# Image-Processing-Systems-Laboratory/DeepInPainting

Measured on AMD Instinct MI355X. Metric: train images/sec at 256x256, batch 8/GPU, 1/2/4/8 MI355X; IPSR layer ms, higher is better.
Workload: dtype f32; 1 GPU; BASELINE config 2: 256x256 synthetic images, 128x128 centre mask (M=256 of N=1024 feature positions), batch 8/GPU, fp32, full IPSR training step; global_batch=8, parallelism=dp1, dropout=True, conv_math=fp32, vgg16=seeded random init (no pretrained weights offline)

## Files before the change

deepinpainting_amd/csrc/winograd.hip:

```cpp
#include <type_traits>

#include "ipsr_common.h"

namespace ipsr {

typedef float f32x16 __attribute__((ext_vector_type(16)));
typedef const __attribute__((address_space(1))) void* gptr_t;
typedef __attribute__((address_space(3))) void* lptr_t;

constexpr int WG_BM = 128, WG_BN = 128, WG_BK = 16, WG_NBUF = 4, WG_THREADS = 256;

struct WinoSplit {
    int nsplit, sps, xi_split, nsplit_t, sps_t;
    int nxi = 36;
    __host__ __device__ int slabs() const { return xi_split >= nxi ? nsplit : (xi_split <= 0 ? nsplit_t : (nsplit > nsplit_t ? nsplit : nsplit_t)); }
    __host__ __device__ int of(int xi) const { return xi < xi_split ? nsplit : nsplit_t; }
    __host__ __device__ int head_xi() const { return xi_split < nxi ? xi_split : nxi; }
    __host__ int workgroups(int tiles_per_xi) const { return tiles_per_xi * (head_xi() * nsplit + (nxi - head_xi()) * nsplit_t); }
};

__device__ __forceinline__ void wino_load_sum(const float* __restrict__ M, const WinoSplit sp, size_t plane, size_t off, float m[6][6])
{
#pragma unroll
    for (int i = 0; i < 6; ++i)
// ... 1104 lines not shown
        for (int j = 0; j < 3; ++j) {
            const int yy = 3 * ty + i, xx = 3 * tx + j;
            e[i][j] = (live && yy < Ho && xx < Wo) ? ld1(dp, (size_t)yy * Wo + xx) : 0.0f;
        }
    float w[6][3], v[6][6];
#pragma unroll
    for (int j = 0; j < 3; ++j) {
        const float col[3] = {e[0][j], e[1][j], e[2][j]};
        float o[6];
        wino_g(col, o);
#pragma unroll
        for (int i = 0; i < 6; ++i) w[i][j] = o[i];
    }
#pragma unroll
    for (int i = 0; i < 6; ++i) wino_g(w[i], v[i]);
    op_emit<true, MODE>(smem, v, ix, Et, Kp, Tp);
    }
};

__global__ void __launch_bounds__(256) wino_wrw_output4_kernel(const float* __restrict__ Mw, WinoSplit split, int K, int C, int Kp, int Cp,
                                                               float* __restrict__ dW)
{
    const int c = blockIdx.x * 256 + threadIdx.x, k = blockIdx.y;
    if (c >= C) return;
    float m[6][6];
    const size_t plane = (size_t)Kp * Cp;
    wino_load_sum(Mw, split, plane, (size_t)k * Cp + c, m);
    float w[4][6], o[4][4];
#pragma unroll
    for (int j = 0; j < 6; ++j) {
        const float col[6] = {m[0][j], m[1][j], m[2][j], m[3][j], m[4][j], m[5][j]};
        float r4[4];
        wino_at(col, r4);
#pragma unroll
        for (int i = 0; i < 4; ++i) w[i][j] = r4[i];
    }
#pragma unroll
    for (int i = 0; i < 4; ++i) wino_at(w[i], o[i]);
    float4* dst = reinterpret_cast<float4*>(dW + ((size_t)k * C + c) * 16);
#pragma unroll
    for (int i = 0; i < 4; ++i) dst[i] = make_float4(o[i][0], o[i][1], o[i][2], o[i][3]);
}

struct DilGrid { int Ho, Wo, Gy, Gx; };
static DilGrid dil_grid(int geom, int mode, int H, int W)
{
    const int Ho = geom == 0 ? H / 2 : H - 1, Wo = geom == 0 ? W / 2 : W - 1;
    return DilGrid{Ho, Wo, (geom == 1 && mode == 1) ? H : Ho, (geom == 1 && mode == 1) ? W : Wo};
}

static int dil_plan(int geom, int mode, int B, int Cin, int H, int W, int Cout, WinoGemmPlan* p, int math)
{
    if (geom != 0 && geom != 1) return fail(IPSR_ERR_INVALID, "4x4 winograd: geometry %d", geom);
    if (geom == 0 && ((H | W) & 1)) return fail(IPSR_ERR_UNSUPPORTED, "dilated winograd: odd extent %dx%d", H, W);
    if (geom == 1 && (H < 4 || W < 4)) return fail(IPSR_ERR_UNSUPPORTED, "4x4 winograd: extent %dx%d below the kernel", H, W);
    const DilGrid g = dil_grid(geom, mode, H, W);
    wino_plan_tiles(p, B, (g.Gy + 2) / 3, (g.Gx + 2) / 3);
    const int red = mode == 0 ? Cin : Cout;
    if (mode != 2 && red % WG_BK != 0)
        return fail(IPSR_ERR_UNSUPPORTED, "4x4 winograd: %d reduction channels are not a multiple of %d", red, WG_BK);
    if (mode == 2) wino_plan_gemm(p, Cout, round_up_bn(Cin), p->Tp, math);
    else wino_plan_gemm(p, mode == 0 ? Cout : Cin, p->Tp, red, math);
    return IPSR_OK;
}

size_t winograd_dil_ws_bytes(int geom, int mode, int B, int Cin, int H, int W, int Cout)
{
    return wino_ws_bytes([&](WinoGemmPlan* p, int math) { return dil_plan(geom, mode, B, Cin, H, W, Cout, p, math); });
}

template <bool TMAJOR, int MODE, typename T, typename F>
static void with_window3(int is, const T* x, int B, int C, int H, int W, int off, const WinoGemmPlan& p, int Cp, void* V, F&& f)
{
    const dim3 grid = op_grid(TMAJOR, MODE, p.Tp, TMAJOR ? Cp : C);
    if (is == 2) f(WinoWindow<3, 2, TMAJOR, MODE, T>{x, B, C, H, W, off, p.TY, p.TX, p.Tp, Cp, V}, grid);
    else f(WinoWindow<3, 1, TMAJOR, MODE, T>{x, B, C, H, W, off, p.TY, p.TX, p.Tp, Cp, V}, grid);
}

int launch_winograd_dil(int geom, int mode, const void* a, const void* b2, void* out, int B, int Cin, int H, int W, int Cout,
                        void* ws, size_t ws_bytes, hipStream_t st, ConvArith ar = ConvArith{0, false, false})
{
    WinoGemmPlan p;
    WinoBufs m;
    if (int rc = dil_plan(geom, mode, B, Cin, H, W, Cout, &p, ar.math)) return rc;
    if (int rc = wino_launch_head("4x4 winograd", "", p, ar, ws, ws_bytes, &m)) return rc;
    const DilGrid g = dil_grid(geom, mode, H, W);
    const int Ho = g.Ho, Wo = g.Wo;
    const int xis = geom == 0 ? 2 : 1, xoff = geom == 0 ? -3 : -1;
    if (mode == 0 || mode == 1) {
        const int red = mode == 0 ? Cin : Cout, prod = mode == 0 ? Cout : Cin;
        if (mode == 1 && geom == 0 && hipMemsetAsync(out, 0, (size_t)B * Cin * H * W * (ar.out_bf16 ? 2 : 4), st) != hipSuccess)
            return fail(IPSR_ERR_LAUNCH, "dilated winograd: hipMemsetAsync failed");
        const float* w = static_cast<const float*>(b2);
        with_mode(ar.math, [&](auto M) {
            constexpr int MODE = decltype(M)::value;
            const Wino4Filter<MODE> filt = mode == 0 ? Wino4Filter<MODE>{w, Cin, Cout, p.rows, 16, (long)Cin * 16, 0, m.A}
                                                     : Wino4Filter<MODE>{w, Cout, Cin, p.rows, (long)Cin * 16, 16, 1, m.A};
            const dim3 fgrid = op_grid(false, MODE, p.rows, red);
            with_type(ar.in_bf16, [&](auto* tag) {
                using T = ELEM_T(tag);
                auto go = [&](const auto& win, dim3 grid) { launch_pair(st, win, grid, wino_remap(), filt, fgrid); };
                if (mode == 0) with_window3<false, MODE, T>(xis, static_cast<const T*>(a), B, Cin, H, W, xoff, p, 0, m.B, go);
                else with_window3<false, MODE, T>(1, static_cast<const T*>(a), B, Cout, Ho, Wo, geom == 0 ? -1 : -2, p, 0, m.B, go);
            });
        });
        if (int rc = check_launch("wino_pair_kernel<WinoWindow, Wino4Filter>")) return rc;
        if (int rc = launch_wino_gemm(ar.math, p, m, st, 72.0 * red * prod * p.T)) return rc;
        with_type(ar.out_bf16, [&](auto* tag) {
            using T = ELEM_T(tag);
            if (mode == 0) wino3_output_kernel<T><<<dim3(cdiv(p.T, 256), prod), 256, 0, st>>>(m.M, p.sp, B, Cout, p.rows, Ho, Wo, p.TY, p.TX, p.Tp, Ho, Wo, 1, 0, static_cast<T*>(out));
            else wino3_output_kernel<T><<<dim3(cdiv(p.T, 256), prod), 256, 0, st>>>(m.M, p.sp, B, Cin, p.rows, g.Gy, g.Gx, p.TY, p.TX, p.Tp, H, W,
                                                                                    geom == 0 ? 2 : 1, geom == 0 ? 1 : 0, static_cast<T*>(out));
        });
        return check_launch("wino3_output_kernel");
    }
    with_mode(ar.math, [&](auto M) {
        constexpr int MODE = decltype(M)::value;
        with_type(ar.in_bf16, [&](auto* tag) {
            using T = ELEM_T(tag);
            const WinoWrwTile3<MODE, T> tile{static_cast<const T*>(b2), B, Cout, Ho, Wo, p.TY, p.TX, p.Tp, p.rows, m.A};
            with_window3<true, MODE, T>(xis, static_cast<const T*>(a), B, Cin, H, W, xoff, p, p.cols, m.B, [&](const auto& win, dim3 grid) {
                launch_pair_wrw(st, tile, op_grid(true, MODE, p.Tp, p.rows), win, grid, MODE != 3);
            });
        });
    });
    if (int rc = check_launch("wino_pair_kernel<WinoWrwTile3, WinoWindow>")) return rc;
    if (int rc = launch_wino_gemm(ar.math, p, m, st, 72.0 * p.T * Cout * Cin)) return rc;
    wino_wrw_output4_kernel<<<dim3(cdiv(Cin, 256), Cout), 256, 0, st>>>(m.M, p.sp, Cout, Cin, p.rows, p.cols, static_cast<float*>(out));
    return check_launch("wino_wrw_output4_kernel");
}

__device__ __forceinline__ void wino_g2(const float g[2], float u[6])
{
    u[0] = 0.25f * g[0];
    u[1] = (-1.0f / 6.0f) * (g[0] + g[1]);
    u[2] = (-1.0f / 6.0f) * (g[0] - g[1]);
    u[3] = (1.0f / 24.0f) * g[0] + (1.0f / 12.0f) * g[1];
    u[4] = (1.0f / 24.0f) * g[0] - (1.0f / 12.0f) * g[1];
    u[5] = g[1];
}
__device__ __forceinline__ void wino_at5(const float m[6], float y[5])
{
    y[0] = m[0] + m[1] + m[2] + m[3] + m[4];
    y[1] = m[1] - m[2] + 2.0f * m[3] - 2.0f * m[4];
    y[2] = m[1] + m[2] + 4.0f * m[3] + 4.0f * m[4];
    y[3] = m[1] - m[2] + 8.0f * m[3] - 8.0f * m[4];
    y[4] = m[1] + m[2] + 16.0f * m[3] + 16.0f * m[4] + m[5];
}
__device__ __forceinline__ void wino_g5(const float e[5], float u[6])
{
    u[0] = 0.25f * e[0];
    u[1] = (-1.0f / 6.0f) * (e[0] + e[1] + e[2] + e[3] + e[4]);
    u[2] = (-1.0f / 6.0f) * (e[0] - e[1] + e[2] - e[3] + e[4]);
    u[3] = (1.0f / 24.0f) * e[0] + (1.0f / 12.0f) * e[1] + (1.0f / 6.0f) * e[2] + (1.0f / 3.0f) * e[3] + (2.0f / 3.0f) * e[4];
    u[4] = (1.0f / 24.0f) * e[0] - (1.0f / 12.0f) * e[1] + (1.0f / 6.0f) * e[2] - (1.0f / 3.0f) * e[3] + (2.0f / 3.0f) * e[4];
    u[5] = e[4];
}
__device__ __forceinline__ void wino_at2(const float m[6], float y[2])
{
    y[0] = m[0] + m[1] + m[2] + m[3] + m[4];
    y[1] = m[1] - m[2] + 2.0f * m[3] - 2.0f * m[4] + m[5];
}

struct Wino52Filter {
    const float* W; int Kc, Cf, Qp, form; float* Uout;
    static constexpr int SMEM = 16;
    __device__ __forceinline__ void operator()(unsigned char*, unsigned bx, unsigned by) const
    {
    float* __restrict__ U = Uout;
    const int fast = bx * 256 + threadIdx.x, slow = by;
    const int nfast = form == 0 ? Kc : Cf;
    const int R = form == 0 ? 4 * Cf : Kc, Q = form == 0 ? Kc : 4 * Cf;
    const size_t plane = (size_t)R * Qp;
    if (fast >= nfast) {
        if (form == 0) {
            if (fast < Qp)
                for (int ph = 0; ph < 4; ++ph)
                    for (int xi = 0; xi < 36; ++xi) U[(size_t)xi * plane + (size_t)(ph * Cf + slow) * Qp + fast] = 0.0f;
        } else {
            const int q = Q + (fast - nfast);
            if (q < Qp)
                for (int xi = 0; xi < 36; ++xi) U[(size_t)xi * plane + (size_t)slow * Qp + q] = 0.0f;
        }
        return;
    }
    const int kc = form == 0 ? fast : slow, cf = form == 0 ? slow : fast;
    float w[4][4];
    const float4* wp = reinterpret_cast<const float4*>(W + ((size_t)kc * Cf + cf) * 16);
#pragma unroll
    for (int i = 0; i < 4; ++i) { const float4 v = wp[i]; w[i][0] = v.x; w[i][1] = v.y; w[i][2] = v.z; w[i][3] = v.w; }
#pragma unroll
    for (int ph = 0; ph < 4; ++ph) {
        const int ey = ph >> 1, ex = ph & 1;
        float g[2][2];
#pragma unroll
        for (int a = 0; a < 2; ++a)
#pragma unroll
            for (int b = 0; b < 2; ++b) g[a][b] = form == 0 ? w[2 * a + ey][2 * b + ex] : w[3 - ey - 2 * a][3 - ex - 2 * b];
        float t[6][2], u[6][6];
#pragma unroll
        for (int b = 0; b < 2; ++b) {
            const float col[2] = {g[0][b], g[1][b]};
            float o[6];
            wino_g2(col, o);
#pragma unroll
            for (int i = 0; i < 6; ++i) t[i][b] = o[i];
        }
#pragma unroll
        for (int i = 0; i < 6; ++i) wino_g2(t[i], u[i]);
        const size_t r = form == 0 ? (size_t)ph * Cf + cf : kc, q = form == 0 ? kc : (size_t)ph * Cf + cf;
#pragma unroll
        for (int i = 0; i < 6; ++i)
#pragma unroll
            for (int j = 0; j < 6; ++j) U[(size_t)(i * 6 + j) * plane + r * Qp + q] = u[i][j];
    }
    }
};

template <int NPL>
struct Wino52FilterSplit {
    const float* W; int Kc, Cf, Qp, form; unsigned short* U;
    static constexpr int SMEM = split_stage_elems<NPL>() * 2;
    __device__ __forceinline__ void operator()(unsigned char* smem, unsigned bx, unsigned by) const
    {
    unsigned short* stage = reinterpret_cast<unsigned short*>(smem);
    const int pk = threadIdx.x >> 5, rl = threadIdx.x & 31;
    const int kc = form == 0 ? bx * SPLIT_ROWS + rl : by * 8 + pk;
    const int cf = form == 0 ? by * 8 + pk : bx * SPLIT_ROWS + rl;
    const bool live = kc < Kc && cf < Cf;
    float w[4][4];
    const float4* wp = reinterpret_cast<const float4*>(W + ((size_t)(live ? kc : 0) * Cf + (live ? cf : 0)) * 16);
#pragma unroll
    for (int i = 0; i < 4; ++i) {
        const float4 v = live ? wp[i] : make_float4(0.f, 0.f, 0.f, 0.f);
        w[i][0] = v.x; w[i][1] = v.y; w[i][2] = v.z; w[i][3] = v.w;
    }
#pragma unroll
    for (int ph = 0; ph < 4; ++ph) {
        const int ey = ph >> 1, ex = ph & 1;
        float g[2][2];
#pragma unroll
        for (int a = 0; a < 2; ++a)
#pragma unroll
            for (int b = 0; b < 2; ++b) g[a][b] = form == 0 ? w[2 * a + ey][2 * b + ex] : w[3 - ey - 2 * a][3 - ex - 2 * b];
        float t[6][2], u[6][6];
#pragma unroll
        for (int b = 0; b < 2; ++b) {
            const float col[2] = {g[0][b], g[1][b]};
            float o[6];
            wino_g2(col, o);
#pragma unroll
            for (int i = 0; i < 6; ++i) t[i][b] = o[i];
        }
#pragma unroll
        for (int i = 0; i < 6; ++i) wino_g2(t[i], u[i]);
        if (form == 0) store_split<NPL>(stage, u, pk, rl, U, (size_t)4 * Cf / 8, Qp, (size_t)ph * Cf / 8 + by, (size_t)bx * SPLIT_ROWS);
        else store_split<NPL>(stage, u, pk, rl, U, (size_t)Kc / 8, Qp, by, (size_t)ph * Cf + (size_t)bx * SPLIT_ROWS);
    }
    }
};

template <int IS, bool TMAJOR, int MODE, typename TIN>
struct Wino5Window {
    const TIN* x; int B, C, H, Wd, nphase, TY, TX, Tp, Cp; void* V;
    static constexpr int SMEM = op_smem_bytes<TMAJOR, MODE>();
    __device__ __forceinline__ void operator()(unsigned char* smem, unsigned bx, unsigned by) const
    {
    const int Ctot = nphase * C;
    const OpIdx ix = op_index<TMAJOR, MODE>(bx, by);
    const int t = ix.t, cc = ix.c;
    if (!TMAJOR && MODE == 0 && t >= Tp) return;
    const int T = B * TY * TX;
    const bool live = t < T && cc < Ctot;
    int b = 0, ty = 0, tx = 0, ph = 0, c = 0;
    if (live) { b = t / (TY * TX); const int rem = t - b * TY * TX; ty = rem / TX; tx = rem - ty * TX; ph = cc / C; c = cc - ph * C; }
    const int offy = nphase == 4 ? (ph >> 1) - 1 : -1, offx = nphase == 4 ? (ph & 1) - 1 : -1;
    const TIN* xp = x + ((size_t)b * C + c) * H * Wd;
    float d[6][6];
#pragma unroll
    for (int i = 0; i < 6; ++i) {
        const int yy = IS * (5 * ty + i) + offy;
        const bool yok = live && (unsigned)yy < (unsigned)H;
#pragma unroll
        for (int j = 0; j < 6; ++j) {
            const int xx = IS * (5 * tx + j) + offx;
            d[i][j] = (yok && (unsigned)xx < (unsigned)Wd) ? ld1(xp, (size_t)yy * Wd + xx) : 0.0f;
        }
    }
    float w[6][6], v[6][6];
#pragma unroll
    for (int j = 0; j < 6; ++j) {
        const float col[6] = {d[0][j], d[1][j], d[2][j], d[3][j], d[4][j], d[5][j]};
        float o[6];
        wino_bt(col, o);
#pragma unroll
        for (int i = 0; i < 6; ++i) w[i][j] = o[i];
    }
#pragma unroll
    for (int i = 0; i < 6; ++i) wino_bt(w[i], v[i]);
    op_emit<TMAJOR, MODE>(smem, v, ix, V, TMAJOR ? Cp : Ctot, Tp);
    }
};

__device__ __forceinline__ void wino_at5_2d(const float m[6][6], float o[5][5])
{
    float w[5][6];
#pragma unroll
    for (int j = 0; j < 6; ++j) {
        const float col[6] = {m[0][j], m[1][j], m[2][j], m[3][j], m[4][j], m[5][j]};
        float r5[5];
        wino_at5(col, r5);
#pragma unroll
        for (int i = 0; i < 5; ++i) w[i][j] = r5[i];
    }
#pragma unroll
    for (int i = 0; i < 5; ++i) wino_at5(w[i], o[i]);
}

template <typename TOUT>
__global__ void __launch_bounds__(256) wino5_output_kernel(const float* __restrict__ Mo, WinoSplit split, int B, int K, int Kp, int Ho, int Wo,
                                                           int TY, int TX, int Tp, TOUT* __restrict__ y)
{
    const int t = blockIdx.x * 256 + threadIdx.x, k = blockIdx.y;
    const int T = B * TY * TX;
    if (t >= T) return;
    float m[6][6], o[5][5];
    wino_load_sum(Mo, split, (size_t)Kp * Tp, (size_t)k * Tp + t, m);
    wino_at5_2d(m, o);
    const int b = t / (TY * TX), rem = t - b * TY * TX;
    const int ty = rem / TX, tx = rem - ty * TX;
    TOUT* yp = y + ((size_t)b * K + k) * Ho * Wo;
#pragma unroll
    for (int i = 0; i < 5; ++i)
#pragma unroll
        for (int j = 0; j < 5; ++j) {
            const int oy = 5 * ty + i, ox = 5 * tx + j;
            if (oy < Ho && ox < Wo) st1(yp, (size_t)oy * Wo + ox, o[i][j]);
        }
}

constexpr int W5R_TILES = 64;
template <typename TOUT>
__global__ void __launch_bounds__(256) wino5_output_rows_kernel(const float* __restrict__ Mo, WinoSplit split, int B, int K, int Kp, int nh, int nw,
                                                                int TY, int TX, int Tp, TOUT* __restrict__ y)
{
    __shared__ float blk[W5R_TILES][101];
    __shared__ int org_y[W5R_TILES], org_x[W5R_TILES], org_b[W5R_TILES];
    const int tl = threadIdx.x & 63, ph = threadIdx.x >> 6, ey = ph >> 1, ex = ph & 1;
    const int t0 = blockIdx.x * W5R_TILES, t = t0 + tl, k = blockIdx.y;
    const int T = B * TY * TX;
    if (t < T) {
        float m[6][6], o[5][5];
        wino_load_sum(Mo, split, (size_t)Kp * Tp, (size_t)(ph * K + k) * Tp + t, m);
        wino_at5_2d(m, o);
#pragma unroll
        for (int i = 0; i < 5; ++i)
#pragma unroll
            for (int j = 0; j < 5; ++j) blk[tl][(2 * i - ey + 1) * 10 + (2 * j - ex + 1)] = o[i][j];
        if (ph == 0) {
            const int b = t / (TY * TX), rem = t - b * TY * TX;
            const int ty = rem / TX, tx = rem - ty * TX;
            org_b[tl] = b; org_y[tl] = 10 * ty - 1; org_x[tl] = 10 * tx - 1;
        }
    }
    __syncthreads();
    const int Hy = 2 * nh, Wy = 2 * nw;
    const int ntile = min(W5R_TILES, T - t0);
    for (int e = threadIdx.x; e < 10 * 10 * W5R_TILES; e += 256) {
        const int r = e / (10 * W5R_TILES), xs = e - r * (10 * W5R_TILES);
        const int tile = xs / 10, c = xs - tile * 10;
        if (tile >= ntile) continue;
        const int fy = org_y[tile] + r, fx = org_x[tile] + c;
        if (fy < 0 || fy >= Hy || fx < 0 || fx >= Wy) continue;
        st1(y + ((size_t)org_b[tile] * K + k) * (size_t)Hy * Wy, (size_t)fy * Wy + fx, blk[tile][r * 10 + c]);
    }
}

template <int MODE, typename TIN>
struct WinoWrwTile5 {
    const TIN* dy; int B, K, Ho, Wo, TY, TX, Tp, Kp; void* Et;
    static constexpr int SMEM = op_smem_bytes<true, MODE>();
    __device__ __forceinline__ void operator()(unsigned char* smem, unsigned bx, unsigned by) const
    {
    const OpIdx ix = op_index<true, MODE>(bx, by);
    const int t = ix.t, k = ix.c, T = B * TY * TX;
    const bool live = t < T && k < K;
    int b = 0, ty = 0, tx = 0;
    if (live) { b = t / (TY * TX); const int rem = t - b * TY * TX; ty = rem / TX; tx = rem - ty * TX; }
    const TIN* dp = dy + ((size_t)b * K + (live ? k : 0)) * Ho * Wo;
    float e[5][5];
#pragma unroll
    for (int i = 0; i < 5; ++i)
#pragma unroll
        for (int j = 0; j < 5; ++j) {
            const int yy = 5 * ty + i, xx = 5 * tx + j;
            e[i][j] = (live && yy < Ho && xx < Wo) ? ld1(dp, (size_t)yy * Wo + xx) : 0.0f;
        }
    float w[6][5], v[6][6];
#pragma unroll
    for (int j = 0; j < 5; ++j) {
        const float col[5] = {e[0][j], e[1][j], e[2][j], e[3][j], e[4][j]};
        float o[6];
        wino_g5(col, o);
#pragma unroll
        for (int i = 0; i < 6; ++i) w[i][j] = o[i];
    }
#pragma unroll
    for (int i = 0; i < 6; ++i) wino_g5(w[i], v[i]);
    op_emit<true, MODE>(smem, v, ix, Et, Kp, Tp);
    }
};

__global__ void __launch_bounds__(256) wino_wrw_output2_kernel(const float* __restrict__ Mw, WinoSplit split, int Kc, int Cf, int Kp, int Cp,
                                                               float* __restrict__ dW)
{
    const int cf = blockIdx.x * 256 + threadIdx.x, kc = blockIdx.y, ph = blockIdx.z;
    if (cf >= Cf) return;
    float m[6][6], w[2][6], o[2][2];
    wino_load_sum(Mw, split, (size_t)Kp * Cp, (size_t)kc * Cp + (size_t)ph * Cf + cf, m);
#pragma unroll
    for (int j = 0; j < 6; ++j) {
        const float col[6] = {m[0][j], m[1][j], m[2][j], m[3][j], m[4][j], m[5][j]};
        float r2[2];
        wino_at2(col, r2);
        w[0][j] = r2[0]; w[1][j] = r2[1];
    }
    wino_at2(w[0], o[0]);
    wino_at2(w[1], o[1]);
    const int ey = ph >> 1, ex = ph & 1;
    float* dst = dW + ((size_t)kc * Cf + cf) * 16;
#pragma unroll
    for (int a = 0; a < 2; ++a)
#pragma unroll
        for (int b = 0; b < 2; ++b) dst[(2 * a + ey) * 4 + 2 * b + ex] = o[a][b];
}

static int s2_plan(int mode, int B, int Kc, int Cf, int nh, int nw, WinoGemmPlan* p, int math)
{
    if (mode < 0 || mode > 2) return fail(IPSR_ERR_INVALID, "4x4 stride-2 winograd: mode %d", mode);
    wino_plan_tiles(p, B, mode == 1 ? (nh + 5) / 5 : (nh + 4) / 5, mode == 1 ? (nw + 5) / 5 : (nw + 4) / 5);
    const int red = mode == 0 ? 4 * Cf : Kc;
    if (mode != 2 && red % WG_BK != 0)
        return fail(IPSR_ERR_UNSUPPORTED, "4x4 stride-2 winograd: reduction length %d is not a multiple of %d", red, WG_BK);
    if (mode == 2) wino_plan_gemm(p, Kc, round_up_bn(4 * Cf), p->Tp, math);
    else wino_plan_gemm(p, mode == 0 ? Kc : 4 * Cf, p->Tp, red, math);
    return IPSR_OK;
}

size_t winograd_s2_ws_bytes(int mode, int B, int Kc, int Cf, int nh, int nw)
{
    return wino_ws_bytes([&](WinoGemmPlan* p, int math) { return s2_plan(mode, B, Kc, Cf, nh, nw, p, math); });
}

int launch_winograd_s2(int mode, const void* a, const void* b2, void* out, int B, int Kc, int Cf, int nh, int nw,
                       void* ws, size_t ws_bytes, hipStream_t st, ConvArith ar = ConvArith{0, false, false})
{
    WinoGemmPlan p;
    WinoBufs m;
    if (int rc = s2_plan(mode, B, Kc, Cf, nh, nw, &p, ar.math)) return rc;
    if (int rc = wino_launch_head("4x4 stride-2 winograd", "", p, ar, ws, ws_bytes, &m)) return rc;
    if (ar.math && ((mode == 0 && Cf % 8 != 0) || (mode == 1 && (Cf % SPLIT_ROWS != 0 || p.rows != 4 * Cf || Kc % 8 != 0)))) ar.math = 0;
    const int remap = wino_remap();
    if (mode == 0 || mode == 1) {
        const float* w = static_cast<const float*>(b2);
        with_mode(ar.math, [&](auto M) {
            constexpr int MODE = decltype(M)::value;
            with_type(ar.in_bf16, [&](auto* tag) {
                using T = ELEM_T(tag);
                const dim3 wgrid = op_grid(false, MODE, p.Tp, p.red);
                auto go = [&](const auto& filt, dim3 fgrid) {
                    auto pair = [&](const auto& win) {
                        if constexpr (MODE == 0) launch_pair<8>(st, win, wgrid, remap, filt, fgrid);
                        else launch_two(st, win, wgrid, remap, filt, fgrid);
                    };
                    if (mode == 0) pair(Wino5Window<2, false, MODE, T>{static_cast<const T*>(a), B, Cf, 2 * nh, 2 * nw, 4, p.TY, p.TX, p.Tp, 0, m.B});
                    else pair(Wino5Window<1, false, MODE, T>{static_cast<const T*>(a), B, Kc, nh, nw, 1, p.TY, p.TX, p.Tp, 0, m.B});
                };
                if constexpr (MODE == 0)
                    go(Wino52Filter{w, Kc, Cf, p.rows, mode, m.A}, mode == 0 ? dim3(cdiv(p.rows, 256), Cf) : dim3(cdiv(Cf + (p.rows - 4 * Cf), 256), Kc));
                else
                    go(Wino52FilterSplit<MODE>{w, Kc, Cf, p.rows, mode, reinterpret_cast<unsigned short*>(m.A)},
                       mode == 0 ? dim3(p.rows / SPLIT_ROWS, Cf / 8) : dim3(Cf / SPLIT_ROWS, Kc / 8));
            });
        });
        if (int rc = check_launch("wino_pair_kernel<Wino5Window, Wino52Filter>")) return rc;
        if (int rc = launch_wino_gemm(ar.math, p, m, st, 72.0 * p.red * (mode == 0 ? Kc : 4 * Cf) * p.T)) return rc;
        with_type(ar.out_bf16, [&](auto* tag) {
            using T = ELEM_T(tag);
            if (mode == 0) wino5_output_kernel<T><<<dim3(cdiv(p.T, 256), Kc), 256, 0, st>>>(m.M, p.sp, B, Kc, p.rows, nh, nw, p.TY, p.TX, p.Tp, static_cast<T*>(out));
            else wino5_output_rows_kernel<T><<<dim3(cdiv(p.T, W5R_TILES), Cf), 256, 0, st>>>(m.M, p.sp, B, Cf, p.rows, nh, nw, p.TY, p.TX, p.Tp, static_cast<T*>(out));
        });
        return check_launch("wino5_output_kernel");
    }
    with_mode(ar.math, [&](auto M) {
        constexpr int MODE = decltype(M)::value;
        with_type(ar.in_bf16, [&](auto* tag) {
            using T = ELEM_T(tag);
            launch_pair_wrw(st, WinoWrwTile5<MODE, T>{static_cast<const T*>(b2), B, Kc, nh, nw, p.TY, p.TX, p.Tp, p.rows, m.A}, op_grid(true, MODE, p.Tp, p.rows),
                            Wino5Window<2, true, MODE, T>{static_cast<const T*>(a), B, Cf, 2 * nh, 2 * nw, 4, p.TY, p.TX, p.Tp, p.cols, m.B}, op_grid(true, MODE, p.Tp, p.cols),
                            MODE != 3);
        });
    });
    if (int rc = check_launch("wino_pair_kernel<WinoWrwTile5, Wino5Window>")) return rc;
    if (int rc = launch_wino_gemm(ar.math, p, m, st, 72.0 * p.T * Kc * 4 * Cf)) return rc;
    wino_wrw_output2_kernel<<<dim3(cdiv(Cf, 256), Kc, 4), 256, 0, st>>>(m.M, p.sp, Kc, Cf, p.rows, p.cols, static_cast<float*>(out));
    return check_launch("wino_wrw_output2_kernel");
}

}

using namespace ipsr;

extern "C" {

int ipsr_debug_force_wino_split(int nsplit, int xi_split, int nsplit_t)
{
    if (nsplit == 0 && xi_split == 0 && nsplit_t == 0) { g_force_split[0] = g_force_split[1] = g_force_split[2] = 0; return IPSR_OK; }
    if (nsplit < 1 || nsplit_t < 1 || xi_split < 1 || xi_split > 36) return fail(IPSR_ERR_INVALID, "ipsr_debug_force_wino_split: bad split %d,%d,%d", nsplit, xi_split, nsplit_t);
    g_force_split[0] = nsplit; g_force_split[1] = xi_split; g_force_split[2] = nsplit_t;
    return IPSR_OK;
}

int ipsr_wino_gemm_split(int rows, int cols, int reduction, int* out5)
{
    if (!out5 || rows < 1 || cols < 1 || reduction < 1 || rows % WG_BM || cols % WG_BN || reduction % WG_BK)
        return fail(IPSR_ERR_INVALID, "ipsr_wino_gemm_split: rows / cols must be multiples of 128 and the reduction of 16");
    const WinoSplit sp = wino_choose_split(36 * (rows / WG_BM) * (cols / WG_BN), reduction / WG_BK, (size_t)36 * rows * cols * 4);
    out5[0] = sp.nsplit; out5[1] = sp.sps; out5[2] = sp.xi_split; out5[3] = sp.nsplit_t; out5[4] = sp.sps_t;
    return IPSR_OK;
}

size_t ipsr_conv3x3_winograd_workspace_bytes(int op, int B, int Cin, int H, int W, int Cout)
{
    if (op < 0 || op > 3 || B < 1 || Cin < 1 || Cout < 1 || H < 1 || W < 1) return 0;
    const bool fwd = op == 0 || op == 2;
    return winograd_ws_bytes(B, fwd ? Cin : Cout, fwd ? Cout : Cin, H, W);
}

static int arith_from(const char* who, int math, int io, ConvArith* ar)
{
    if ((math != 0 && math != 2 && math != 3) || io < 0 || io > 3)
        return fail(IPSR_ERR_INVALID, "%s: math %d (0 = fp32 MFMA, 2 = split bf16 x3, 3 = split bf16 x6) / io %d (bit 0: bf16 activations in, bit 1: out)", who, math, io);
    ar->math = math; ar->in_bf16 = (io & 1) != 0; ar->out_bf16 = (io & 2) != 0;
    return IPSR_OK;
}

int ipsr_conv3x3_winograd_mp(int op, const void* in, const float* weight, const float* bias, int epilogue, float* filter_cache,
                             int filter_cache_valid, void* out, int B, int Cin, int H, int W, int Cout, int math, int io,
                             void* ws, size_t ws_bytes, void* stream)
{
    if (!in || !weight || !out || !ws) return fail(IPSR_ERR_INVALID, "ipsr_conv3x3_winograd: null pointer");
    if (op < 0 || op > 3 || B < 1 || Cin < 1 || Cout < 1 || H < 1 || W < 1) return fail(IPSR_ERR_INVALID, "ipsr_conv3x3_winograd: bad argument");
    if ((reinterpret_cast<uintptr_t>(ws) & 15u) || (reinterpret_cast<uintptr_t>(out) & 15u) || (reinterpret_cast<uintptr_t>(filter_cache) & 15u))
        return fail(IPSR_ERR_INVALID, "ipsr_conv3x3_winograd: out / workspace / filter_cache must be 16-byte aligned");
    ConvArith ar;
    if (int rc = arith_from("ipsr_conv3x3_winograd_mp", math, io, &ar)) return rc;
    if (reinterpret_cast<uintptr_t>(in) & (ar.in_bf16 ? 7u : 15u))
        return fail(IPSR_ERR_INVALID, "ipsr_conv3x3_winograd: in must be aligned to four elements");
    hipStream_t st = static_cast<hipStream_t>(stream);
    switch (op) {
        case 0:
            return launch_winograd(in, weight, out, B, Cin, Cout, H, W, 9, (long)Cin * 9, 0, ws, ws_bytes, st, bias, epilogue, filter_cache, filter_cache_valid, ar);
        case 1:
            return launch_winograd(in, weight, out, B, Cout, Cin, H, W, (long)Cin * 9, 9, 1, ws, ws_bytes, st, bias, epilogue, filter_cache, filter_cache_valid, ar);
        case 2:
            return launch_winograd(in, weight, out, B, Cin, Cout, H, W, (long)Cout * 9, 9, 1, ws, ws_bytes, st, bias, epilogue, filter_cache, filter_cache_valid, ar);
        default:
            return launch_winograd(in, weight, out, B, Cout, Cin, H, W, 9, (long)Cout * 9, 0, ws, ws_bytes, st, bias, epilogue, filter_cache, filter_cache_valid, ar);
    }
}

int ipsr_conv3x3_winograd(int op, const float* in, const float* weight, float* out, int B, int Cin, int H, int W, int Cout,
                          void* ws, size_t ws_bytes, void* stream)
{
    return ipsr_conv3x3_winograd_mp(op, in, weight, nullptr, 0, nullptr, 0, out, B, Cin, H, W, Cout, 0, 0, ws, ws_bytes, stream);
}

size_t ipsr_conv3x3_winograd_filter_floats(int op, int Cin, int Cout)
{
    if (op < 0 || op > 3 || Cin < 1 || Cout < 1) return 0;
    const bool fwd = op == 0 || op == 2;
    return winograd_filter_floats(fwd ? Cin : Cout, fwd ? Cout : Cin);
}

int ipsr_conv3x3_winograd_ex(int op, const float* in, const float* weight, const float* bias, int epilogue, float* filter_cache,
                             int filter_cache_valid, float* out, int B, int Cin, int H, int W, int Cout,
                             void* ws, size_t ws_bytes, void* stream)
{
    return ipsr_conv3x3_winograd_mp(op, in, weight, bias, epilogue, filter_cache, filter_cache_valid, out, B, Cin, H, W, Cout, 0, 0, ws, ws_bytes, stream);
}

size_t ipsr_conv4x4_winograd_workspace_bytes(int geom, int mode, int B, int Cin, int H, int W, int Cout)
{
    if (geom < 0 || geom > 1 || mode < 0 || mode > 2 || B < 1 || Cin < 1 || Cout < 1 || H < 2 || W < 2) return 0;
    return winograd_dil_ws_bytes(geom, mode, B, Cin, H, W, Cout);
}

int ipsr_conv4x4_winograd_mp(int geom, int mode, const void* a, const void* b, void* out, int B, int Cin, int H, int W, int Cout,
                             int math, int io, void* ws, size_t ws_bytes, void* stream)
{
    if (!a || !b || !out || !ws) return fail(IPSR_ERR_INVALID, "ipsr_conv4x4_winograd: null pointer");
    if (geom < 0 || geom > 1 || mode < 0 || mode > 2 || B < 1 || Cin < 1 || Cout < 1 || H < 2 || W < 2)
        return fail(IPSR_ERR_INVALID, "ipsr_conv4x4_winograd: bad argument");
    if ((reinterpret_cast<uintptr_t>(ws) & 15u) || (reinterpret_cast<uintptr_t>(out) & 15u))
        return fail(IPSR_ERR_INVALID, "ipsr_conv4x4_winograd: out / workspace must be 16-byte aligned");
    ConvArith ar;
    if (int rc = arith_from("ipsr_conv4x4_winograd_mp", math, io, &ar)) return rc;
    return launch_winograd_dil(geom, mode, a, b, out, B, Cin, H, W, Cout, ws, ws_bytes, static_cast<hipStream_t>(stream), ar);
}

int ipsr_conv4x4_winograd(int geom, int mode, const float* a, const float* b, float* out, int B, int Cin, int H, int W, int Cout,
                          void* ws, size_t ws_bytes, void* stream)
{
    return ipsr_conv4x4_winograd_mp(geom, mode, a, b, out, B, Cin, H, W, Cout, 0, 0, ws, ws_bytes, stream);
}

size_t ipsr_conv4x4_dilated_winograd_workspace_bytes(int mode, int B, int Cin, int H, int W, int Cout)
{
    return ipsr_conv4x4_winograd_workspace_bytes(0, mode, B, Cin, H, W, Cout);
}

int ipsr_conv4x4_dilated_winograd(int mode, const float* a, const float* b, float* out, int B, int Cin, int H, int W, int Cout,
                                  void* ws, size_t ws_bytes, void* stream)
{
    return ipsr_conv4x4_winograd(0, mode, a, b, out, B, Cin, H, W, Cout, ws, ws_bytes, stream);
}

size_t ipsr_conv4x4s2_winograd_workspace_bytes(int mode, int B, int Kc, int Cf, int nh, int nw)
{
    if (mode < 0 || mode > 2 || B < 1 || Kc < 1 || Cf < 1 || nh < 1 || nw < 1) return 0;
    return winograd_s2_ws_bytes(mode, B, Kc, Cf, nh, nw);
}

int ipsr_conv4x4s2_winograd_mp(int mode, const void* a, const void* b, void* out, int B, int Kc, int Cf, int nh, int nw,
                               int math, int io, void* ws, size_t ws_bytes, void* stream)
{
    if (!a || !b || !out || !ws) return fail(IPSR_ERR_INVALID, "ipsr_conv4x4s2_winograd: null pointer");
    if (mode < 0 || mode > 2 || B < 1 || Kc < 1 || Cf < 1 || nh < 1 || nw < 1) return fail(IPSR_ERR_INVALID, "ipsr_conv4x4s2_winograd: bad argument");
    if ((reinterpret_cast<uintptr_t>(ws) & 15u) || (reinterpret_cast<uintptr_t>(out) & 15u))
        return fail(IPSR_ERR_INVALID, "ipsr_conv4x4s2_winograd: out / workspace must be 16-byte aligned");
    if (mode != 2 && (reinterpret_cast<uintptr_t>(b) & 15u))
        return fail(IPSR_ERR_INVALID, "ipsr_conv4x4s2_winograd: the weight must be 16-byte aligned");
    ConvArith ar;
    if (int rc = arith_from("ipsr_conv4x4s2_winograd_mp", math, io, &ar)) return rc;
    return launch_winograd_s2(mode, a, b, out, B, Kc, Cf, nh, nw, ws, ws_bytes, static_cast<hipStream_t>(stream), ar);
}

int ipsr_conv4x4s2_winograd(int mode, const float* a, const float* b, float* out, int B, int Kc, int Cf, int nh, int nw,
                            void* ws, size_t ws_bytes, void* stream)
{
    return ipsr_conv4x4s2_winograd_mp(mode, a, b, out, B, Kc, Cf, nh, nw, 0, 0, ws, ws_bytes, stream);
}

size_t ipsr_conv3x3_winograd_wrw_workspace_bytes(int transposed, int B, int Cin, int H, int W, int Cout)
{
    if (B < 1 || Cin < 1 || Cout < 1 || H < 1 || W < 1) return 0;
    return transposed ? winograd_wrw_ws_bytes(B, Cin, Cout, H, W) : winograd_wrw_ws_bytes(B, Cout, Cin, H, W);
}

int ipsr_conv3x3_winograd_wrw_mp(int transposed, const void* x, const void* dy, float* dw, int B, int Cin, int H, int W, int Cout,
                                 int math, int io, void* ws, size_t ws_bytes, void* stream)
{
    if (!x || !dy || !dw || !ws) return fail(IPSR_ERR_INVALID, "ipsr_conv3x3_winograd_wrw: null pointer");
    if (B < 1 || Cin < 1 || Cout < 1 || H < 1 || W < 1) return fail(IPSR_ERR_INVALID, "ipsr_conv3x3_winograd_wrw: bad argument");
    if (reinterpret_cast<uintptr_t>(ws) & 15u) return fail(IPSR_ERR_INVALID, "ipsr_conv3x3_winograd_wrw: workspace must be 16-byte aligned");
    ConvArith ar;
    if (int rc = arith_from("ipsr_conv3x3_winograd_wrw_mp", math, io, &ar)) return rc;
    hipStream_t st = static_cast<hipStream_t>(stream);
    if (transposed) return launch_winograd_wrw(x, dy, dw, B, Cin, Cout, H, W, ws, ws_bytes, st, ar);
    return launch_winograd_wrw(dy, x, dw, B, Cout, Cin, H, W, ws, ws_bytes, st, ar);
}

int ipsr_conv3x3_winograd_wrw(int transposed, const float* x, const float* dy, float* dw, int B, int Cin, int H, int W, int Cout,
                              void* ws, size_t ws_bytes, void* stream)
{
    return ipsr_conv3x3_winograd_wrw_mp(transposed, x, dy, dw, B, Cin, H, W, Cout, 0, 0, ws, ws_bytes, stream);
}

}
```

Baseline: 357.8 images/sec.

## Stage stride-2 Winograd input windows through LDS with vectorized row loads

Adds a Wino5WindowRows input transform that cooperatively loads contiguous image rows with float4 loads into shared memory. The rows are de-interleaved by parity, then each thread reads its 6x6 phase window from LDS. The goal is to replace the scattered per-element global gathers of the existing stride-2 window transform in the fp32 forward and weight-gradient paths. In exchange it adds shared-memory use, extra barriers and segment bookkeeping. It only runs when the width is a multiple of 4 and the input is 16-byte aligned.

```diff
diff --git a/deepinpainting_amd/csrc/winograd.hip b/deepinpainting_amd/csrc/winograd.hip
--- a/deepinpainting_amd/csrc/winograd.hip
+++ b/deepinpainting_amd/csrc/winograd.hip
@@ -1430,6 +1430,127 @@
     }
 };
 
+template <bool TMAJOR>
+struct Wino5WindowRows {
+    const float* x; int B, C, H, Wd, TY, TX, Tp, Cp; float* V;
+    static constexpr int R = TMAJOR ? 4 : 64;
+    static constexpr int NCH = TMAJOR ? 16 : 1;
+    static constexpr int NI = TMAJOR ? 6 : 3;
+    static constexpr int NROW = 2 * NI;
+    static constexpr int PITCH = 6 * R;
+    static constexpr int CHS = NROW * 2 * PITCH + (TMAJOR ? 1 : 0);
+    static constexpr int SMEM = NCH * CHS * 4 + (TMAJOR ? 0 : R * 2);
+    static dim3 grid(int Tp, int C) { return dim3(Tp / R, C / NCH); }
+    __device__ __forceinline__ void operator()(unsigned char* smem, unsigned bx, unsigned by) const
+    {
+    float* rows = reinterpret_cast<float*>(smem);
+    const int tid = threadIdx.x;
+    const int q = TMAJOR ? tid >> 6 : tid & 63, ph = TMAJOR ? (tid >> 4) & 3 : tid >> 6, cl = TMAJOR ? tid & 15 : 0;
+    const int ey = ph >> 1, ex = ph & 1;
+    const int T = B * TY * TX, t0 = bx * R, t = t0 + q, c0 = by * NCH;
+    const bool live = t < T;
+    const int g0 = t0 / TX, g1 = (t0 + R - 1) / TX;
+    const int nseg = min(g1, B * TY - 1) - g0 + 1;
+    const int sg = live ? t / TX - g0 : 0;
+    const float* mine = rows + cl * CHS + ex * PITCH + 5 * q + sg;
+    unsigned short* seg_b = reinterpret_cast<unsigned short*>(smem + NCH * CHS * 4);
+    if (!TMAJOR) {
+        if (live && ph == 0 && (q == 0 || t == (g0 + sg) * TX)) seg_b[sg] = (unsigned short)((g0 + sg) / TY);
+        __syncthreads();
+    }
+    float d[6][6];
+#pragma unroll
+    for (int i0 = 0; i0 < 6; i0 += NI) {
+        if (i0) __syncthreads();
+        if constexpr (TMAJOR) {
+            const int vq = tid & 15, ch = tid >> 4;
+            for (int s = 0; s < nseg; ++s) {
+                const int g = g0 + s, b = g / TY, ty = g - b * TY;
+                const int txa = s == 0 ? t0 - g0 * TX : 0, txb = g == g1 ? t0 + R - 1 - g1 * TX : TX - 1;
+                const int xlo = 10 * txa - 1, xhi = 10 * txb + 10, col4 = ((xlo >> 2) + vq) * 4, y0 = 10 * ty - 1;
+                if (col4 > xhi) continue;
+                const bool inmap = (unsigned)col4 < (unsigned)Wd;
+                const float* img = x + ((size_t)b * C + c0 + ch) * H * Wd;
+                float4 val[NROW];
+#pragma unroll
+                for (int k = 0; k < NROW; ++k)
+                    val[k] = (inmap && (unsigned)(y0 + k) < (unsigned)H) ? ld4(img + (size_t)(y0 + k) * Wd, (size_t)col4 >> 2) : make_float4(0.f, 0.f, 0.f, 0.f);
+#pragma unroll
+                for (int e = 0; e < 4; ++e) {
+                    const int xx = col4 + e, m = xx + 1;
+                    if (xx < xlo || xx > xhi) continue;
+                    float* dst = rows + ch * CHS + 5 * (g * TX - t0) + s + (m & 1) * PITCH + (m >> 1);
+#pragma unroll
+                    for (int k = 0; k < NROW; ++k) {
+                        const float e4[4] = {val[k].x, val[k].y, val[k].z, val[k].w};
+                        dst[k * 2 * PITCH] = e4[e];
+                    }
+                }
+            }
+        } else {
+            constexpr int UNROLL = 2;
+            const int NV = min((10 * TX >> 2) + 2, (10 * R + 4) / 4 + 1);
+            const int nitem = nseg * NROW * NV;
+            for (int w0 = tid; w0 < nitem; w0 += 256 * UNROLL) {
+                float4 val[UNROLL];
+                int dst[UNROLL], col4[UNROLL], xlo[UNROLL], xhi[UNROLL];
+#pragma unroll
+                for (int u = 0; u < UNROLL; ++u) {
+                    const int w = w0 + u * 256;
+                    const int row = (unsigned)w / (unsigned)NV, v = w - row * NV, rr = row % NROW, s = row / NROW;
+                    const bool on = w < nitem;
+                    const int g = g0 + s, b = on ? seg_b[s] : 0, ty = g - b * TY;
+                    const int txa = s == 0 ? t0 - g0 * TX : 0, txb = g == g1 ? t0 + R - 1 - g1 * TX : TX - 1;
+                    xlo[u] = 10 * txa - 1;
+                    xhi[u] = on ? 10 * txb + 10 : xlo[u] - 1;
+                    col4[u] = ((xlo[u] >> 2) + v) * 4;
+                    dst[u] = rr * 2 * PITCH + 5 * (g * TX - t0) + s;
+                    const int yy = 10 * ty + 2 * i0 - 1 + rr;
+                    const bool in = col4[u] <= xhi[u] && (unsigned)yy < (unsigned)H && (unsigned)col4[u] < (unsigned)Wd;
+                    val[u] = in ? ld4(x + (((size_t)b * C + c0) * H + yy) * Wd, (size_t)col4[u] >> 2) : make_float4(0.f, 0.f, 0.f, 0.f);
+                }
+#pragma unroll
+                for (int u = 0; u < UNROLL; ++u) {
+                    const float e4[4] = {val[u].x, val[u].y, val[u].z, val[u].w};
+#pragma unroll
+                    for (int e = 0; e < 4; ++e) {
+                        const int xx = col4[u] + e, m = xx + 1;
+                        if (xx >= xlo[u] && xx <= xhi[u]) rows[dst[u] + (m & 1) * PITCH + (m >> 1)] = e4[e];
+                    }
+                }
+            }
+        }
+        __syncthreads();
+#pragma unroll
+        for (int i = 0; i < NI; ++i)
+#pragma unroll
+            for (int j = 0; j < 6; ++j) d[i0 + i][j] = live ? mine[(2 * i + ey) * 2 * PITCH + j] : 0.0f;
+    }
+    float w[6][6], v[6][6];
+#pragma unroll
+    for (int j = 0; j < 6; ++j) {
+        const float col[6] = {d[0][j], d[1][j], d[2][j], d[3][j], d[4][j], d[5][j]};
+        float o[6];
+        wino_bt(col, o);
+#pragma unroll
+        for (int i = 0; i < 6; ++i) w[i][j] = o[i];
+    }
+#pragma unroll
+    for (int i = 0; i < 6; ++i) wino_bt(w[i], v[i]);
+    const size_t plane = TMAJOR ? (size_t)Tp * Cp : (size_t)4 * C * Tp;
+    float* out = V + (TMAJOR ? (size_t)t * Cp + ph * C + c0 + cl : ((size_t)ph * C + c0) * Tp + t);
+#pragma unroll
+    for (int i = 0; i < 6; ++i)
+#pragma unroll
+        for (int j = 0; j < 6; ++j) out[(size_t)(i * 6 + j) * plane] = v[i][j];
+    }
+};
+
+static bool wino_rows_staged(const void* x, int B, int Wd)
+{
+    return (Wd & 3) == 0 && (reinterpret_cast<uintptr_t>(x) & 15u) == 0 && B <= 65535 && !debug_option(5);
+}
+
 __device__ __forceinline__ void wino_at5_2d(const float m[6][6], float o[5][5])
 {
     float w[5][6];
@@ -1601,6 +1722,12 @@
                         if constexpr (MODE == 0) launch_pair<8>(st, win, wgrid, remap, filt, fgrid);
                         else launch_two(st, win, wgrid, remap, filt, fgrid);
                     };
+                    if constexpr (MODE == 0 && std::is_same<T, float>::value) {
+                        if (mode == 0 && wino_rows_staged(a, B, 2 * nw)) {
+                            using Rows = Wino5WindowRows<false>;
+                            return launch_pair<8>(st, Rows{static_cast<const float*>(a), B, Cf, 2 * nh, 2 * nw, p.TY, p.TX, p.Tp, 0, m.B}, Rows::grid(p.Tp, Cf), remap, filt, fgrid);
+                        }
+                    }
                     if (mode == 0) pair(Wino5Window<2, false, MODE, T>{static_cast<const T*>(a), B, Cf, 2 * nh, 2 * nw, 4, p.TY, p.TX, p.Tp, 0, m.B});
                     else pair(Wino5Window<1, false, MODE, T>{static_cast<const T*>(a), B, Kc, nh, nw, 1, p.TY, p.TX, p.Tp, 0, m.B});
                 };
@@ -1624,6 +1751,13 @@
         constexpr int MODE = decltype(M)::value;
         with_type(ar.in_bf16, [&](auto* tag) {
             using T = ELEM_T(tag);
+            if constexpr (MODE == 0 && std::is_same<T, float>::value) {
+                if (Cf % 16 == 0 && p.cols == 4 * Cf && wino_rows_staged(a, B, 2 * nw)) {
+                    using Rows = Wino5WindowRows<true>;
+                    return launch_pair_wrw(st, WinoWrwTile5<0, float>{static_cast<const float*>(b2), B, Kc, nh, nw, p.TY, p.TX, p.Tp, p.rows, m.A}, op_grid(true, 0, p.Tp, p.rows),
+                                           Rows{static_cast<const float*>(a), B, Cf, 2 * nh, 2 * nw, p.TY, p.TX, p.Tp, p.cols, m.B}, Rows::grid(p.Tp, Cf), true);
+                }
+            }
             launch_pair_wrw(st, WinoWrwTile5<MODE, T>{static_cast<const T*>(b2), B, Kc, nh, nw, p.TY, p.TX, p.Tp, p.rows, m.A}, op_grid(true, MODE, p.Tp, p.rows),
                             Wino5Window<2, true, MODE, T>{static_cast<const T*>(a), B, Cf, 2 * nh, 2 * nw, 4, p.TY, p.TX, p.Tp, p.cols, m.B}, op_grid(true, MODE, p.Tp, p.cols),
                             MODE != 3);
```

Measured after the change: 360.8 images/sec, median of 6. No clear change (+0.8%).
